# lmcinnes/pynndescent

Measured on AMD Instinct MI355X. Metric: index build: points indexed/sec (recall@10 vs brute force reported alongside), higher is better.
Workload: dtype f32

## Files before the change

### pynndescent_amd/csrc/rpforest.hip

```cpp
#include <atomic>
#include <chrono>

#include "common.h"
#include "state.h"

#define RP_EPS 1e-8f

static constexpr int SCAN_ITEMS = 8;
static constexpr int SCAN_BLOCK = 256;
static constexpr int SCAN_TILE = SCAN_ITEMS * SCAN_BLOCK;

__global__ void k_forest_init(int32_t *__restrict__ perm, int32_t *__restrict__ pos_seg, uint8_t *__restrict__ leaf_flag,
                              int32_t *__restrict__ inv, int64_t n, int64_t P, int splittable) {
    int64_t g = (int64_t)blockIdx.x * blockDim.x + threadIdx.x;
    if (g >= P) return;
    int64_t t = g / n;
    int64_t i = g - t * n;
    perm[g] = (int32_t)i;
    inv[g] = splittable ? (int32_t)t : -1;
    pos_seg[g] = splittable ? (int32_t)t : -1;
    leaf_flag[g] = (!splittable && i == 0) ? 1 : 0;
}
__global__ void k_forest_init_segs(int32_t *__restrict__ seg_start, int32_t *__restrict__ seg_len, int n_trees,
                                   int64_t n) {
// ... 1027 lines not shown
                    const float band = rp_band(xnorm, rx, hnorm, rh);
                    if (RP_IN_BAND(m, band)) {
                        const float4 *h4 = (const float4 *)(node_hf + (int64_t)node[u] * hs);
                        float e = 0.0f;
#pragma unroll
                        for (int q = 0; q < NC; q++) {
                            const int c = sub + 4 * q;
                            e = rp_dot4f(xa[q], h4[2 * c], e);
                            e = rp_dot4f(xb[q], h4[2 * c + 1], e);
                        }
                        m = rp_quad_sum(e) + off;
                    }
                    const int64_t slot = (int64_t)(t0 + u) * n + i;
                    int side;
                    if (fabsf(m) < RP_EPS) side = (int)(nnd_hash3(seed ^ 0x5bd1e995u, (uint32_t)slot, (uint32_t)depth) & 1u);
                    else side = m > 0.0f ? 0 : 1;
                    const int nxt = (int)(side ? meta[u].w : meta[u].z);
                    if (nxt <= -2) {
                        if (sub == 0) {
                            const int cell = -2 - nxt;
                            cell_of[slot] = cell;
                            rk[u] = atomicAdd(&cell_count[cell], 1);
                        }
                        node[u] = -1;
                    } else {
                        node[u] = nxt;
                    }
                }
            }
            if (sub == 0) {
#pragma unroll
                for (int u = 0; u < TB; u++)
                    if (t0 + u < n_trees) rank_of[(int64_t)(t0 + u) * n + i] = rk[u];
            }
        }
    }
}

#define RP_GLOBAL_TAG 0x40000000

__global__ __launch_bounds__(256) void k_top_heap(const unsigned char *__restrict__ pack, int rec, int dp, const int32_t *__restrict__ roots,
                                                  int L1, unsigned char *__restrict__ top_rec, int32_t *__restrict__ top_node,
                                                  int32_t *__restrict__ bucket_root) {
    __shared__ int32_t hn[256];
    const int t = blockIdx.x, nslots = 1 << L1, r16 = rec >> 4;
    if (threadIdx.x == 0) {
        hn[0] = -1;
        hn[1] = roots[t];
    }
    __syncthreads();
    for (int l = 0; l < L1; l++) {
        for (int sl = (1 << l) + threadIdx.x; sl < (2 << l); sl += blockDim.x) {
            const int nd = hn[sl];
            int c0 = -1, c1 = -1;
            if (nd >= 0) {
                const uint4 meta = *(const uint4 *)(pack + (int64_t)nd * rec + 2 * dp);
                c0 = (int)meta.z;
                c1 = (int)meta.w;
            }
            hn[2 * sl] = c0 >= 0 ? c0 : -1;
            hn[2 * sl + 1] = c1 >= 0 ? c1 : -1;
        }
        __syncthreads();
    }
    for (int q = threadIdx.x; q < nslots * r16; q += blockDim.x) {
        const int sl = q / r16, wd = q - sl * r16;
        const int nd = hn[sl];
        if (nd >= 0) ((uint4 *)(top_rec + (size_t)t * nslots * rec))[q] = ((const uint4 *)(pack + (int64_t)nd * rec))[wd];
    }
    for (int sl = threadIdx.x; sl < nslots; sl += blockDim.x) {
        top_node[t * nslots + sl] = hn[sl];
        bucket_root[t * nslots + sl] = hn[nslots + sl];
    }
}

__device__ __forceinline__ float rp_pair_sum(float v) {
    return v + __int_as_float(__builtin_amdgcn_update_dpp(0, __float_as_int(v), 0xB1, 0xF, 0xF, false));
}
template <int NC>
__device__ __forceinline__ float rp_exact_pair(const float *__restrict__ xrow, const float *__restrict__ h, int sub) {
    const float4 *x4 = (const float4 *)xrow;
    const float4 *h4 = (const float4 *)h;
    float ea = 0.0f, eb = 0.0f;
#pragma unroll
    for (int q = 0; q < NC; q++) {
        const int c = sub + 4 * q, c2 = sub + 2 + 4 * q;
        ea = rp_dot4f(x4[2 * c], h4[2 * c], ea);
        ea = rp_dot4f(x4[2 * c + 1], h4[2 * c + 1], ea);
        eb = rp_dot4f(x4[2 * c2], h4[2 * c2], eb);
        eb = rp_dot4f(x4[2 * c2 + 1], h4[2 * c2 + 1], eb);
    }
    ea = rp_pair_sum(ea);
    eb = rp_pair_sum(eb);
    return ea + eb;
}

template <int NC>
__global__ __launch_bounds__(1024) void k_route_top(const float *__restrict__ xp, const uint16_t *__restrict__ xh,
                                                    const float2 *__restrict__ nr, int metric, int dp, int64_t n, int64_t row_lo,
                                                    int64_t nrows, int tg0, int tgn, int L1, const unsigned char *__restrict__ top_rec,
                                                    const int32_t *__restrict__ top_node, const float *__restrict__ node_hf, int hs,
                                                    uint32_t seed, int32_t *__restrict__ cell_count, int32_t *__restrict__ cell_of,
                                                    int32_t *__restrict__ rank_of, int32_t *__restrict__ code,
                                                    int32_t *__restrict__ bucket_count, const float *__restrict__ scal) {
    extern __shared__ __attribute__((aligned(16))) unsigned char top_tab[];
    constexpr int NC2 = 2 * NC;
    const int rec = 2 * dp + 16, nslots = 1 << L1;
    const float inv_s2 = scal[1];
    int32_t *hist = (int32_t *)(top_tab + (size_t)tgn * nslots * rec);
    int32_t *tnode = hist + tgn * nslots;
    {
        const uint4 *src = (const uint4 *)(top_rec + (size_t)tg0 * nslots * rec);
        uint4 *dst = (uint4 *)top_tab;
        const int total = tgn * nslots * (rec >> 4);
        for (int q = threadIdx.x; q < total; q += blockDim.x) dst[q] = src[q];
        for (int q = threadIdx.x; q < tgn * nslots; q += blockDim.x) {
            hist[q] = 0;
            tnode[q] = top_node[tg0 * nslots + q];
        }
    }
    __syncthreads();
    const int sub = threadIdx.x & 1;
    const int ppb = blockDim.x >> 1;
    for (int64_t r0 = (int64_t)blockIdx.x * ppb; r0 < nrows; r0 += (int64_t)gridDim.x * ppb) {
        const int64_t r = r0 + (threadIdx.x >> 1);
        const bool on = r < nrows;
        const int64_t i = row_lo + (on ? r : 0);
        uint4 xq[NC2];
        {
            const uint4 *row = (const uint4 *)(xh + i * dp);
#pragma unroll
            for (int q = 0; q < NC2; q++) xq[q] = row[sub + 2 * q];
        }
        const float2 nrv = nr[i];
        const float xnorm = nnd_metric_unit(metric) ? nrv.x : sqrtf(nrv.x);
        const float bA = nrv.y + RP_ACC * xnorm, bB = xnorm + nrv.y;
        for (int tl = 0; tl < tgn; tl++) {
            const int t = tg0 + tl;
            const int64_t slot = (int64_t)t * n + i;
            int hidx = 1, rk = 0;
            bool fin = false;
            for (int depth = 0; depth < L1; depth++) {
                if (!__ballot(!fin)) break;
                const uint4 *r8 = (const uint4 *)(top_tab + ((size_t)tl * nslots + (fin ? 1 : hidx)) * rec);
                uint4 p[NC2];
#pragma unroll
                for (int q = 0; q < NC2; q++) p[q] = r8[sub + 2 * q];
                const uint4 meta = r8[dp >> 3];
                float acc = 0.0f;
#pragma unroll
                for (int q = 0; q < NC2; q++) acc = rp_dot8(xq[q], p[q], acc);
                if (fin) continue;
                const float off = __uint_as_float(meta.x), hnorm = __uint_as_float(meta.y & 0xFFFF0000u), rh = __uint_as_float(meta.y << 16);
                float m = rp_pair_sum(acc) * inv_s2 + off;
                const float band = hnorm * bA + rh * bB + RP_EPS;
                if (RP_IN_BAND(m, band))
                    m = rp_exact_pair<NC>(xp + i * dp, node_hf + (int64_t)tnode[tl * nslots + hidx] * hs, sub) + off;
                int side;
                if (fabsf(m) < RP_EPS) side = (int)(nnd_hash3(seed ^ 0x5bd1e995u, (uint32_t)slot, (uint32_t)depth) & 1u);
                else side = m > 0.0f ? 0 : 1;
                const int nxt = (int)(side ? meta.w : meta.z);
                if (nxt <= -2) {
                    if (sub == 0 && on) {
                        const int cell = -2 - nxt;
                        cell_of[(int64_t)t * nrows + r] = cell;
                        rk = atomicAdd(&cell_count[cell], 1);
                    }
                    fin = true;
                } else {
                    hidx = 2 * hidx + side;
                }
            }
            if (sub == 0 && on) {
                const int64_t o = (int64_t)t * nrows + r;
                if (fin) {
                    rank_of[o] = rk;
                    code[o] = -1;
                } else {
                    const int b = hidx - nslots;
                    code[o] = t * nslots + b;
                    atomicAdd(&hist[tl * nslots + b], 1);
                }
            }
        }
    }
    __syncthreads();
    for (int q = threadIdx.x; q < tgn * nslots; q += blockDim.x)
        if (hist[q]) atomicAdd(&bucket_count[tg0 * nslots + q], hist[q]);
}

__global__ __launch_bounds__(256) void k_bucket_prefix(const int32_t *__restrict__ bucket_count, int nb, int chunk,
                                                       int32_t *__restrict__ bucket_start, int2 *__restrict__ items,
                                                       int32_t *__restrict__ n_items, int max_items) {
    __shared__ int pa[256], pi[256];
    const int per = (nb + 255) / 256;
    const int b0 = threadIdx.x * per < nb ? threadIdx.x * per : nb, b1 = b0 + per < nb ? b0 + per : nb;
    int sa = 0, si = 0;
    for (int b = b0; b < b1; b++) {
        const int c = bucket_count[b];
        sa += c;
        si += (c + chunk - 1) / chunk;
    }
    pa[threadIdx.x] = sa;
    pi[threadIdx.x] = si;
    __syncthreads();
    if (threadIdx.x == 0) {
        int ra = 0, ri = 0;
        for (int q = 0; q < 256; q++) {
            const int va = pa[q], vi = pi[q];
            pa[q] = ra;
            pi[q] = ri;
            ra += va;
            ri += vi;
        }
        bucket_start[nb] = ra;
        n_items[0] = ri < max_items ? ri : max_items;
    }
    __syncthreads();
    int ra = pa[threadIdx.x], ri = pi[threadIdx.x];
    for (int b = b0; b < b1; b++) {
        const int c = bucket_count[b];
        bucket_start[b] = ra;
        ra += c;
        const int nc = (c + chunk - 1) / chunk;
        for (int j = 0; j < nc; j++)
            if (ri + j < max_items) items[ri + j] = make_int2(b, j);
        ri += nc;
    }
}

__global__ __launch_bounds__(256) void k_bucket_scatter(const int32_t *__restrict__ code, int64_t nrows, int64_t row_lo, int L1,
                                                        const int32_t *__restrict__ bucket_start, int32_t *__restrict__ bucket_cursor,
                                                        int32_t *__restrict__ bucket_rows, const float2 *__restrict__ nr, int metric,
                                                        uint32_t *__restrict__ bucket_ab) {
    __shared__ int cnt[256], base[256];
    const int t = blockIdx.y, nslots = 1 << L1;
    for (int q = threadIdx.x; q < nslots; q += 256) cnt[q] = 0;
    __syncthreads();
    const int64_t r0 = (int64_t)blockIdx.x * 4096;
    int myc[16], myr[16];
#pragma unroll
    for (int it = 0; it < 16; it++) {
        const int64_t r = r0 + it * 256 + threadIdx.x;
        const int c = r < nrows ? code[(int64_t)t * nrows + r] : -1;
        myc[it] = c;
        myr[it] = c >= 0 ? atomicAdd(&cnt[c - t * nslots], 1) : 0;
    }
    __syncthreads();
    for (int q = threadIdx.x; q < nslots; q += 256) base[q] = cnt[q] ? atomicAdd(&bucket_cursor[t * nslots + q], cnt[q]) : 0;
    __syncthreads();
#pragma unroll
    for (int it = 0; it < 16; it++) {
        const int c = myc[it];
        if (c < 0) continue;
        const int64_t r = r0 + it * 256 + threadIdx.x;
        const int at = bucket_start[c] + base[c - t * nslots] + myr[it];
        bucket_rows[at] = (int32_t)(row_lo + r);
        const float2 nrv = nr[row_lo + r];
        const float xnm = nnd_metric_unit(metric) ? nrv.x : sqrtf(nrv.x);
        bucket_ab[at] = (rp_bf16_up(nrv.y + RP_ACC * xnm) << 16) | rp_bf16_up(xnm + nrv.y);
    }
}

__global__ __launch_bounds__(64) void k_bucket_tables(const unsigned char *__restrict__ pack, int rec, int dp,
                                                      const int32_t *__restrict__ bucket_root, int R, int32_t *__restrict__ bt_cnt,
                                                      int32_t *__restrict__ bt_node, int32_t *__restrict__ bt_child,
                                                      unsigned char *__restrict__ bt_rec, int32_t *__restrict__ bt_cell) {
    const int b = blockIdx.x, lane = nnd_lane();
    int32_t *nodes = bt_node + (size_t)b * R;
    int32_t *child = bt_child + (size_t)b * R * 2;
    int32_t *cells = bt_cell + (size_t)b * (R + 8);
    const int root = bucket_root[b];
    if (root < 0) {
        if (lane == 0) bt_cnt[b] = 0;
        return;
    }
    int ccount = 0;
    __shared__ int32_t q_nodes[1024];
    if (lane == 0) q_nodes[0] = root;
    int count = 1, lb = 0, le = 1;
    nnd_wave_lds_sync();
    while (lb < le) {
        for (int i0 = lb; i0 < le; i0 += 64) {
            const int idx = i0 + lane;
            int c0 = -1, c1 = -1;
            if (idx < le) {
                const uint4 meta = *(const uint4 *)(pack + (int64_t)q_nodes[idx] * rec + 2 * dp);
                c0 = (int)meta.z;
                c1 = (int)meta.w;
            }
            const unsigned long long m0 = __ballot(idx < le && c0 >= 0), m1 = __ballot(idx < le && c1 >= 0);
            const int p0 = count + nnd_prefix_popc(m0), p1 = count + __popcll(m0) + nnd_prefix_popc(m1);
            const unsigned long long z0 = __ballot(idx < le && c0 <= -2), z1 = __ballot(idx < le && c1 <= -2);
            const int l0 = ccount + nnd_prefix_popc(z0), l1 = ccount + __popcll(z0) + nnd_prefix_popc(z1);
            ccount += __popcll(z0) + __popcll(z1);
            if (idx < le) {
                int k0 = c0, k1 = c1;
                if (c0 <= -2) { cells[l0] = -2 - c0; k0 = -2 - l0; }
                if (c1 <= -2) { cells[l1] = -2 - c1; k1 = -2 - l1; }
                if (c0 >= 0) {
                    if (p0 < R) { q_nodes[p0] = c0; k0 = p0; } else k0 = c0 + RP_GLOBAL_TAG;
                }
                if (c1 >= 0) {
                    if (p1 < R) { q_nodes[p1] = c1; k1 = p1; } else k1 = c1 + RP_GLOBAL_TAG;
                }
                child[2 * idx] = k0;
                child[2 * idx + 1] = k1;
            }
            count += __popcll(m0) + __popcll(m1);
            if (count > R) count = R;
            nnd_wave_lds_sync();
        }
        lb = le;
        le = count;
    }
    for (int i = lane; i < count; i += 64) nodes[i] = q_nodes[i];
    if (lane == 0) bt_cnt[b] = count;
    __threadfence_block();
    const int r16 = rec >> 4;
    uint4 *dst = (uint4 *)(bt_rec + (size_t)b * R * rec);
    for (int q = lane; q < count * r16; q += 64) {
        const int sl = q / r16, wd = q - sl * r16;
        uint4 v = ((const uint4 *)(pack + (int64_t)q_nodes[sl] * rec))[wd];
        if (wd == r16 - 1) {
            v.z = (uint32_t)child[2 * sl];
            v.w = (uint32_t)child[2 * sl + 1];
        }
        dst[q] = v;
    }
}

template <int NC>
__global__ __launch_bounds__(1024) void k_route_bucket(const float *__restrict__ xp, const uint16_t *__restrict__ xh,
                                                      const float2 *__restrict__ nr, int metric, int dp, int64_t n, int64_t row_lo,
                                                      int64_t nrows, int L1, int chunk, const unsigned char *__restrict__ pack,
                                                      const float *__restrict__ node_hf, int hs, const int2 *__restrict__ items,
                                                      const int32_t *__restrict__ n_items, const int32_t *__restrict__ bucket_start,
                                                      const int32_t *__restrict__ bucket_rows, const uint32_t *__restrict__ bucket_ab, int R,
                                                      const int32_t *__restrict__ bt_cnt, const int32_t *__restrict__ bt_node,
                                                      const unsigned char *__restrict__ bt_rec, const int32_t *__restrict__ bt_cell, uint32_t seed, int32_t *__restrict__ cell_count,
                                                      int32_t *__restrict__ cell_of, int32_t *__restrict__ rank_of,
                                                      const float *__restrict__ scal) {
    extern __shared__ __attribute__((aligned(16))) unsigned char sub_tab[];
    constexpr int NC2 = 2 * NC;
    const int rec = 2 * dp + 16, r16 = rec >> 4;
    const float inv_s2 = scal[1];
    int32_t *lcnt = (int32_t *)(sub_tab + (size_t)R * rec);
    int32_t *lbase = lcnt + (R + 8);
    int32_t *lcell = lbase + (R + 8);
    uint32_t *rowbuf = (uint32_t *)(lcell + (R + 8));
    const int sub = threadIdx.x & 1, ppb = blockDim.x >> 1, pair = threadIdx.x >> 1;
    const int ni = n_items[0];
#ifndef NND_ROUTE_CONTIG
    const int item0 = (int)blockIdx.x, item1 = ni, istep = (int)gridDim.x;
#else
    const int per = (ni + (int)gridDim.x - 1) / (int)gridDim.x;
    const int item0 = (int)blockIdx.x * per, item1 = item0 + per < ni ? item0 + per : ni, istep = 1;
#endif
    int cur_b = -1;
    for (int item = item0; item < item1; item += istep) {
        const int2 it = items[item];
        const int b = it.x;
        if (b != cur_b) {
            __syncthreads();
            const int cnt = bt_cnt[b];
            const uint4 *src = (const uint4 *)(bt_rec + (size_t)b * R * rec);
            for (int q = threadIdx.x; q < cnt * r16; q += blockDim.x) ((uint4 *)sub_tab)[q] = src[q];
            for (int q = threadIdx.x; q < R + 8; q += blockDim.x) {
                lcnt[q] = 0;
                lcell[q] = q <= cnt ? bt_cell[(size_t)b * (R + 8) + q] : 0;
            }
            cur_b = b;
            __syncthreads();
        }
        const int t = b >> L1;
        const int base = bucket_start[b] + it.y * chunk;
        int cnt_rows = bucket_start[b + 1] - base;
        if (cnt_rows > chunk) cnt_rows = chunk;
        for (int r0 = 0; r0 < cnt_rows; r0 += ppb) {
            const int idx = r0 + pair;
            const bool on = idx < cnt_rows;
            const int64_t pi = bucket_rows[base + (on ? idx : 0)];
            const uint32_t ab = bucket_ab[base + (on ? idx : 0)];
            uint4 xq[NC2];
            {
                const uint4 *row = (const uint4 *)(xh + pi * dp);
#pragma unroll
                for (int q = 0; q < NC2; q++) xq[q] = row[sub + 2 * q];
            }
            const float bA = __uint_as_float(ab & 0xFFFF0000u), bB = __uint_as_float(ab << 16);
            const int64_t slot = (int64_t)t * n + pi;
            int cur = on ? 0 : -1;
            int rk = -1;
            for (int depth = L1;; depth++) {
                if (!__ballot(cur >= 0)) break;
                uint4 p[NC2], meta;
                const bool glob = cur >= RP_GLOBAL_TAG;
                if (glob) {
                    const uint4 *r8 = (const uint4 *)(pack + (int64_t)(cur - RP_GLOBAL_TAG) * rec);
#pragma unroll
                    for (int q = 0; q < NC2; q++) p[q] = r8[sub + 2 * q];
                    meta = r8[dp >> 3];
                    if ((int)meta.z >= 0) meta.z += RP_GLOBAL_TAG;
                    if ((int)meta.w >= 0) meta.w += RP_GLOBAL_TAG;
                } else {
                    const uint4 *r8 = (const uint4 *)(sub_tab + (size_t)(cur >= 0 ? cur : 0) * rec);
#pragma unroll
                    for (int q = 0; q < NC2; q++) p[q] = r8[sub + 2 * q];
                    meta = r8[dp >> 3];
                }
                float acc = 0.0f;
#pragma unroll
                for (int q = 0; q < NC2; q++) acc = rp_dot8(xq[q], p[q], acc);
                if (cur < 0) continue;
                const float off = __uint_as_float(meta.x), hnorm = __uint_as_float(meta.y & 0xFFFF0000u), rh = __uint_as_float(meta.y << 16);
                float m = rp_pair_sum(acc) * inv_s2 + off;
                const float band = hnorm * bA + rh * bB + RP_EPS;
                if (RP_IN_BAND(m, band)) {
                    const int nd = glob ? cur - RP_GLOBAL_TAG : bt_node[(size_t)b * R + cur];
                    m = rp_exact_pair<NC>(xp + pi * dp, node_hf + (int64_t)nd * hs, sub) + off;
                }
                int side;
                if (fabsf(m) < RP_EPS) side = (int)(nnd_hash3(seed ^ 0x5bd1e995u, (uint32_t)slot, (uint32_t)depth) & 1u);
                else side = m > 0.0f ? 0 : 1;
                const int nxt = (int)(side ? meta.w : meta.z);
                if (nxt <= -2) {
                    if (sub == 0) {
                        const int cell = -2 - nxt;
                        if (glob) {
                            const int64_t o = (int64_t)t * nrows + (pi - row_lo);
                            cell_of[o] = cell;
                            rank_of[o] = atomicAdd(&cell_count[cell], 1);
                        } else {
                            rk = (cell << 16) | atomicAdd(&lcnt[cell], 1);
                        }
                    }
                    cur = -1;
                } else {
                    cur = nxt;
                }
            }
            if (sub == 0 && on) rowbuf[idx] = (uint32_t)rk;
        }
        __syncthreads();
        for (int q = threadIdx.x; q < R + 8; q += blockDim.x) {
            const int c = lcnt[q];
            if (c) {
                lbase[q] = atomicAdd(&cell_count[lcell[q]], c);
                lcnt[q] = 0;
            }
        }
        __syncthreads();
        for (int idx = threadIdx.x; idx < cnt_rows; idx += blockDim.x) {
            const uint32_t v = rowbuf[idx];
            if (v == 0xFFFFFFFFu) continue;
            const int lc = (int)(v >> 16);
            const int64_t o = (int64_t)t * nrows + (bucket_rows[base + idx] - row_lo);
            cell_of[o] = lcell[lc];
            rank_of[o] = lbase[lc] + (int)(v & 0xFFFFu);
        }
        __syncthreads();
    }
}

__global__ void k_cell_depths(const uint8_t *__restrict__ leaf_flag, const int32_t *__restrict__ leafscan,
                              const int32_t *__restrict__ leaf_depth, int64_t ps, int32_t *__restrict__ cell_depth) {
    const int64_t g = (int64_t)blockIdx.x * blockDim.x + threadIdx.x;
    if (g < ps && leaf_flag[g]) cell_depth[leafscan[g]] = leaf_depth[g];
}

__global__ void k_cell_lists(const int32_t *__restrict__ cell_count, const int32_t *__restrict__ cell_start,
                             const int32_t *__restrict__ cell_depth, int n_cells, int fin_small, int fin_max,
                             int32_t *__restrict__ small_list, int32_t *__restrict__ fin_start, int32_t *__restrict__ fin_len,
                             int32_t *__restrict__ fin_depth, int32_t *__restrict__ big_start, int32_t *__restrict__ big_len,
                             int32_t *__restrict__ big_depth, int64_t list_stride,
                             long long *__restrict__ counts ) {
    const int c = blockIdx.x * blockDim.x + threadIdx.x;
    const int len = c < n_cells ? cell_count[c] : 0;
    const int cls = len <= 0 ? -1 : (len <= fin_small ? 2 : (len <= fin_max ? 0 : 1));
#pragma unroll
    for (int k = 0; k < 3; k++) {
        const unsigned long long m = __ballot(cls == k);
        if (!m) continue;
        long long base = 0;
        if (nnd_lane() == __builtin_ctzll(m)) base = (long long)atomicAdd((unsigned long long *)&counts[k], (unsigned long long)__popcll(m));
        base = ((long long)__shfl((int)(base >> 32), __builtin_ctzll(m), 64) << 32) | (unsigned)__shfl((int)base, __builtin_ctzll(m), 64);
        if (cls == k) {
            const int64_t idx = base + nnd_prefix_popc(m);
            int32_t *st = k == 2 ? small_list : (k == 0 ? fin_start : big_start);
            int32_t *ln = k == 2 ? small_list + list_stride : (k == 0 ? fin_len : big_len);
            int32_t *dp_ = k == 2 ? small_list + 2 * list_stride : (k == 0 ? fin_depth : big_depth);
            st[idx] = cell_start[c];
            ln[idx] = len;
            dp_[idx] = cell_depth[c];
        }
    }
}

__global__ void k_place(const int32_t *__restrict__ cell_of, const int32_t *__restrict__ rank_of,
                        const int32_t *__restrict__ cell_start, int64_t nrows, int64_t row_lo, int32_t *__restrict__ perm) {
    const int64_t r = (int64_t)blockIdx.x * blockDim.x + threadIdx.x;
    if (r >= nrows) return;
    const int64_t slot = (int64_t)blockIdx.y * nrows + r;
    perm[cell_start[cell_of[slot]] + rank_of[slot]] = (int32_t)(row_lo + r);
}

enum forest_rc { FOREST_OK = 0, FOREST_ERROR = 1, FOREST_FALLBACK = 2 };
static forest_rc forest_fallback(const char *reason) {
    if (nnd_knob("NND_FOREST_DEBUG")) fprintf(stderr, "forest: fallback: %s\n", reason);
    return FOREST_FALLBACK;
}
#define FOREST_HIP_CHECK(expr) NND_HIP_CHECK_AS(expr, #expr, FOREST_ERROR)

static forest_rc run_scan(nnd_ctx *ctx, int mode, const int32_t *pos_seg, uint8_t *bytes, int32_t *total_dev, int64_t P, int64_t n,
                          const int32_t *perm = nullptr) {
    int nb = (int)((P + SCAN_TILE - 1) / SCAN_TILE);
    hipLaunchKernelGGL(k_scan_reduce, dim3(nb), dim3(SCAN_BLOCK), 0, ctx->stream, mode, pos_seg, bytes, P, ctx->scan_blk, perm,
                       ctx->side_pt, n);
    hipLaunchKernelGGL(k_scan_apply<true>, dim3(nb), dim3(SCAN_BLOCK), 0, ctx->stream, mode == 2 ? 0 : mode, pos_seg, bytes, P,
                       ctx->scan_blk, ctx->scan_out, total_dev);
    FOREST_HIP_CHECK(hipGetLastError());
    return FOREST_OK;
}

static forest_rc scan_i32_inplace(nnd_ctx *ctx, int32_t *data, int64_t n, int32_t *total_dev) {
    if (n <= SCAN_TILE) {
        hipLaunchKernelGGL(k_scan_blocks, dim3(1), dim3(256), 0, ctx->stream, data, (int)n, total_dev);
    } else {
        const int nb = (int)((n + SCAN_TILE - 1) / SCAN_TILE);
        hipLaunchKernelGGL(k_scan_i32_reduce, dim3(nb), dim3(SCAN_BLOCK), 0, ctx->stream, data, n, ctx->scan_blk);
        hipLaunchKernelGGL(k_scan_blocks, dim3(1), dim3(256), 0, ctx->stream, ctx->scan_blk, nb, total_dev);
        hipLaunchKernelGGL(k_scan_i32_apply, dim3(nb), dim3(SCAN_BLOCK), 0, ctx->stream, data, n, ctx->scan_blk);
    }
    FOREST_HIP_CHECK(hipGetLastError());
    return FOREST_OK;
}

static forest_rc read_scan_total(nnd_ctx *ctx, int32_t *out) {
    FOREST_HIP_CHECK(hipMemcpyAsync(&ctx->h_pin->scan_total, nnd_scan_total(ctx), sizeof(int32_t), hipMemcpyDeviceToHost, ctx->stream));
    FOREST_HIP_CHECK(nnd_sync_spin(ctx));
    *out = ctx->h_pin->scan_total;
    return FOREST_OK;
}

// ... 239 lines not shown
static forest_rc launch_route(nnd_ctx *ctx, const rp_route_io &io, int n_top, int l_top) {
    auto kern = k_route<NC, TB>;
    const size_t smem = (size_t)n_top * (2 * ctx->dp + 16);
    static bool attr_dev[64] = {false};
    if (!attr_dev[ctx->p.device & 63]) {
        FOREST_HIP_CHECK(hipFuncSetAttribute((const void *)kern, hipFuncAttributeMaxDynamicSharedMemorySize, 72 * 1024));
        attr_dev[ctx->p.device & 63] = true;
    }
    int n_cu = 0;
    if (device_cus(ctx, &n_cu)) return FOREST_ERROR;
    int64_t blocks = (ctx->n + 127) / 128;
    if (blocks > 2 * (int64_t)n_cu) blocks = 2 * (int64_t)n_cu;
    hipLaunchKernelGGL(kern, dim3((unsigned)blocks), dim3(512), smem, ctx->stream, ctx->xp, ctx->nr2, ctx->p.metric, ctx->dp, ctx->n,
                       io.T, io.pack, io.hf, ctx->dp + 4, ctx->tree_seed, io.cell_count, io.cell_of, io.rank_of, n_top, l_top, ctx->mean + ctx->dp);
    FOREST_HIP_CHECK(hipGetLastError());
    return FOREST_OK;
}

static forest_rc route_plain(nnd_ctx *ctx, const rp_route_io &io, const forest_view &v) {
    const int dp = ctx->dp;
    int l_top = 0;
    while (l_top + 1 < (int)v.level_base.size() && v.level_base[l_top + 1] * (2 * dp + 16) <= 72 * 1024) l_top++;
    const int n_top = (int)v.level_base[l_top];
    switch (dp / 32) {
        case 1: return launch_route<1, 4>(ctx, io, n_top, l_top);
        case 2: return launch_route<2, 4>(ctx, io, n_top, l_top);
        case 3: return launch_route<3, 2>(ctx, io, n_top, l_top);
        case 4: return launch_route<4, 2>(ctx, io, n_top, l_top);
        case 5: return launch_route<5, 1>(ctx, io, n_top, l_top);
        case 6: return launch_route<6, 1>(ctx, io, n_top, l_top);
        case 7: return launch_route<7, 1>(ctx, io, n_top, l_top);
        case 8: return launch_route<8, 1>(ctx, io, n_top, l_top);
        default: break;
    }
    return FOREST_FALLBACK;
}

#ifndef NND_ROUTE_L1
#define NND_ROUTE_L1 6
#endif
#ifndef NND_ROUTE_CHUNK
#define NND_ROUTE_CHUNK 2048
#endif
#ifndef NND_ROUTE_RMAX
#define NND_ROUTE_RMAX 384
#endif

struct rp_route_geom {
    int L1, ns, nb, R, chunk, tg;
    int64_t max_items;
    size_t o_top_rec, o_top_node, o_bucket_root, o_bcount, o_bcursor, o_bstart, o_nitems, o_btcnt, o_btnode, o_btchild, o_btrec, o_btcell, o_items, total;
};
static rp_route_geom route_geometry(int dp, int T, int64_t nrows, int64_t n_cells) {
    rp_route_geom g;
    const int rec = 2 * dp + 16;
    g.L1 = NND_ROUTE_L1;
    if (g.L1 < 7 && n_cells / ((int64_t)T << g.L1) > NND_ROUTE_RMAX / 2) g.L1 = 7;
    g.ns = 1 << g.L1;
    g.nb = T * g.ns;
    int64_t r = 6 * n_cells / g.nb + 16;
    const int64_t r_lds = (int64_t)150 * 1024 / rec;
    if (r > NND_ROUTE_RMAX) r = NND_ROUTE_RMAX;
    if (r > r_lds) r = r_lds;
    g.R = (int)(r < 64 ? 64 : r);
    g.chunk = NND_ROUTE_CHUNK;
    g.tg = (int)((size_t)140 * 1024 / ((size_t)g.ns * (rec + 8)));
    if (g.tg < 1) g.tg = 1;
    if (g.tg > T) g.tg = T;
    g.max_items = (int64_t)g.nb + (int64_t)T * nrows / g.chunk + 1;
    size_t at = 0;
    auto take = [&](size_t bytes) { const size_t o = at; at += (bytes + 255) & ~(size_t)255; return o; };
    g.o_top_rec = take((size_t)g.nb * rec);
    g.o_top_node = take(sizeof(int32_t) * g.nb);
    g.o_bucket_root = take(sizeof(int32_t) * g.nb);
    g.o_bcount = take(sizeof(int32_t) * g.nb);
    g.o_bcursor = take(sizeof(int32_t) * g.nb);
    g.o_bstart = take(sizeof(int32_t) * (g.nb + 1));
    g.o_nitems = take(sizeof(int32_t) * 4);
    g.o_btcnt = take(sizeof(int32_t) * g.nb);
    g.o_btnode = take(sizeof(int32_t) * (size_t)g.nb * g.R);
    g.o_btchild = take(sizeof(int32_t) * (size_t)g.nb * g.R * 2);
    g.o_btrec = take((size_t)g.nb * g.R * rec);
    g.o_btcell = take(sizeof(int32_t) * (size_t)g.nb * (g.R + 8));
    g.o_items = take(sizeof(int2) * (size_t)g.max_items);
    g.total = at;
    return g;
}

template <int NC>
static forest_rc launch_route_coherent(nnd_ctx *ctx, const rp_route_io &io, const rp_route_geom &g) {
    const int dp = ctx->dp, rec = 2 * dp + 16, hs = dp + 4;
    unsigned char *ws = ctx->route_ws;
    unsigned char *top_rec = ws + g.o_top_rec;
    int32_t *top_node = (int32_t *)(ws + g.o_top_node), *bucket_root = (int32_t *)(ws + g.o_bucket_root);
    int32_t *bcount = (int32_t *)(ws + g.o_bcount), *bcursor = (int32_t *)(ws + g.o_bcursor), *bstart = (int32_t *)(ws + g.o_bstart);
    int32_t *n_items = (int32_t *)(ws + g.o_nitems), *bt_cnt = (int32_t *)(ws + g.o_btcnt), *bt_node = (int32_t *)(ws + g.o_btnode);
    int32_t *bt_child = (int32_t *)(ws + g.o_btchild);
    unsigned char *bt_rec = ws + g.o_btrec;
    int32_t *bt_cell = (int32_t *)(ws + g.o_btcell);
    int2 *items = (int2 *)(ws + g.o_items);
    auto ktop = k_route_top<NC>;
    auto kbkt = k_route_bucket<NC>;
    static bool attr_dev[64] = {false};
    if (!attr_dev[ctx->p.device & 63]) {
        FOREST_HIP_CHECK(hipFuncSetAttribute((const void *)ktop, hipFuncAttributeMaxDynamicSharedMemorySize, 160 * 1024));
        FOREST_HIP_CHECK(hipFuncSetAttribute((const void *)kbkt, hipFuncAttributeMaxDynamicSharedMemorySize, 160 * 1024));
        attr_dev[ctx->p.device & 63] = true;
    }
    int n_cu = 0;
    if (device_cus(ctx, &n_cu)) return FOREST_ERROR;
    FOREST_HIP_CHECK(hipMemsetAsync(bcount, 0, g.o_bstart - g.o_bcount, ctx->stream));
    hipLaunchKernelGGL(k_top_heap, dim3((unsigned)io.T), dim3(256), 0, ctx->stream, io.pack, rec, dp, io.roots, g.L1, top_rec, top_node,
                       bucket_root);
    hipLaunchKernelGGL(k_bucket_tables, dim3((unsigned)g.nb), dim3(64), 0, ctx->stream, io.pack, rec, dp, bucket_root, g.R, bt_cnt, bt_node,
                       bt_child, bt_rec, bt_cell);
    for (int tg0 = 0; tg0 < io.T; tg0 += g.tg) {
        const int tgn = io.T - tg0 < g.tg ? io.T - tg0 : g.tg;
        const size_t smem = (size_t)tgn * g.ns * (rec + 8);
        int64_t blocks = (io.nrows + 511) / 512;
        if (blocks > n_cu) blocks = n_cu;
        hipLaunchKernelGGL(ktop, dim3((unsigned)blocks), dim3(1024), smem, ctx->stream, ctx->xp, ctx->xh, ctx->nr2, ctx->p.metric, dp, ctx->n, io.row_lo,
                           io.nrows, tg0, tgn, g.L1, top_rec, top_node, io.hf, hs, ctx->tree_seed, io.cell_count, io.cell_of, io.rank_of,
                           io.code, bcount, ctx->mean + ctx->dp);
    }
    hipLaunchKernelGGL(k_bucket_prefix, dim3(1), dim3(256), 0, ctx->stream, bcount, g.nb, g.chunk, bstart, items, n_items, (int)g.max_items);
    hipLaunchKernelGGL(k_bucket_scatter, dim3((unsigned)((io.nrows + 4095) / 4096), (unsigned)io.T), dim3(256), 0, ctx->stream, io.code,
                       io.nrows, io.row_lo, g.L1, bstart, bcursor, io.bucket_rows, ctx->nr2, ctx->p.metric, (uint32_t *)io.bucket_ab);
    const size_t smem2 = (size_t)g.R * rec + sizeof(int32_t) * 3 * (size_t)(g.R + 8) + sizeof(uint32_t) * (size_t)g.chunk;
    int per_cu = 0;
    FOREST_HIP_CHECK(hipOccupancyMaxActiveBlocksPerMultiprocessor(&per_cu, (const void *)kbkt, 1024, smem2));
    if (per_cu < 1) per_cu = 1;
    int64_t blocks2 = (int64_t)n_cu * per_cu;
    if (blocks2 > g.max_items) blocks2 = g.max_items;
    hipLaunchKernelGGL(kbkt, dim3((unsigned)blocks2), dim3(1024), smem2, ctx->stream, ctx->xp, ctx->xh, ctx->nr2, ctx->p.metric, dp, ctx->n,
                       io.row_lo, io.nrows, g.L1, g.chunk, io.pack, io.hf, hs, items, n_items, bstart, io.bucket_rows, (const uint32_t *)io.bucket_ab, g.R, bt_cnt, bt_node,
                       bt_rec, bt_cell, ctx->tree_seed, io.cell_count, io.cell_of, io.rank_of, ctx->mean + ctx->dp);
    FOREST_HIP_CHECK(hipGetLastError());
    return FOREST_OK;
}

static forest_rc route_coherent(nnd_ctx *ctx, const rp_route_io &io) {
    const int dp = ctx->dp;
    if (dp % 32 != 0 || dp > 256 || io.T < 1 || io.T > NND_ROUTE_TREES_MAX) return FOREST_FALLBACK;
    const rp_route_geom g = route_geometry(dp, io.T, io.nrows, io.n_cells);
    if (g.total > ctx->route_ws_cap) {
        FOREST_HIP_CHECK(hipStreamSynchronize(ctx->stream));
        if (ctx->route_ws) { FOREST_HIP_CHECK(hipFree(ctx->route_ws)); ctx->route_ws = nullptr; }
        ctx->route_ws_cap = 0;
        FOREST_HIP_CHECK(hipMalloc((void **)&ctx->route_ws, g.total + g.total / 4));
        ctx->route_ws_cap = g.total + g.total / 4;
    }
    switch (dp / 32) {
        case 1: return launch_route_coherent<1>(ctx, io, g);
        case 2: return launch_route_coherent<2>(ctx, io, g);
        case 3: return launch_route_coherent<3>(ctx, io, g);
        case 4: return launch_route_coherent<4>(ctx, io, g);
        case 5: return launch_route_coherent<5>(ctx, io, g);
        case 6: return launch_route_coherent<6>(ctx, io, g);
        case 7: return launch_route_coherent<7>(ctx, io, g);
        case 8: return launch_route_coherent<8>(ctx, io, g);
        default: break;
    }
    return FOREST_FALLBACK;
}

__global__ void k_iota_i32(int32_t *__restrict__ out, int n, int base) {
    const int i = blockIdx.x * blockDim.x + threadIdx.x;
    if (i < n) out[i] = base + i;
}

static forest_rc forest_tops(nnd_ctx *ctx, forest_view &v, int32_t *n_cells_out) {
    forest_rc rc = forest_levels(ctx, v);
    if (rc) return rc;
    int32_t n_cells = 0;
    if ((rc = run_scan(ctx, 1, nullptr, ctx->leaf_flag, nnd_scan_total(ctx), v.P, v.rows.n)) || (rc = read_scan_total(ctx, &n_cells))) return rc;
    if (n_cells > ctx->cell_cap) return forest_fallback("the recorded trees have more cells than the cell tables hold");
    hipLaunchKernelGGL(k_cell_depths, dim3((unsigned)((v.P + 255) / 256)), dim3(256), 0, ctx->stream, ctx->leaf_flag, ctx->scan_out,
                       ctx->s_leaf_depth, v.P, ctx->cell_depth);
    FOREST_HIP_CHECK(hipGetLastError());
    *n_cells_out = n_cells;
    return FOREST_OK;
}

static forest_rc forest_place_finish(nnd_ctx *ctx, int32_t n_cells, int T, int64_t row_lo, int64_t nrows, const int32_t *cell_of,
                                     const int32_t *rank_of, int64_t P_used, rp_tree_map tm) {
    FOREST_HIP_CHECK(hipMemcpyAsync(ctx->cell_start, ctx->cell_count, sizeof(int32_t) * (size_t)n_cells, hipMemcpyDeviceToDevice, ctx->stream));
    if (scan_i32_inplace(ctx, ctx->cell_start, n_cells, nnd_scan_total(ctx))) return FOREST_ERROR;
    FOREST_HIP_CHECK(hipMemsetAsync(ctx->leaf_flag, 0, (size_t)P_used, ctx->stream));
    long long *counts = ctx->counters + CNT_FIN_COUNT;
    FOREST_HIP_CHECK(hipMemsetAsync(counts, 0, 3 * sizeof(long long), ctx->stream));
    const nnd_work_list fin = nnd_fin_list(ctx), big = nnd_big_list(ctx), small = nnd_small_list(ctx);
    hipLaunchKernelGGL(k_cell_lists, dim3((unsigned)((n_cells + 255) / 256)), dim3(256), 0, ctx->stream, ctx->cell_count, ctx->cell_start,
                       ctx->cell_depth, (int)n_cells, FIN_SMALL, FIN_MAX, small.start, fin.start, fin.len, fin.depth, big.start,
                       big.len, big.depth, small.len - small.start, counts);
    if (cell_of)
        hipLaunchKernelGGL(k_place, dim3((unsigned)((nrows + 255) / 256), (unsigned)T), dim3(256), 0, ctx->stream, cell_of, rank_of,
                           ctx->cell_start, nrows, row_lo, ctx->perm[0]);
    FOREST_HIP_CHECK(hipGetLastError());
    FOREST_HIP_CHECK(hipMemcpyAsync(&ctx->h_pin->n_big, ctx->counters + CNT_BIG_COUNT, 2 * sizeof(long long), hipMemcpyDeviceToHost, ctx->stream));
    FOREST_HIP_CHECK(nnd_sync_spin(ctx));
    const long long n_big = ctx->h_pin->n_big, n_small = ctx->h_pin->n_small;
    if (n_big > ctx->max_segs) return forest_fallback("more over-long cells than the big work list holds");
    if (launch_finishers(ctx, ctx->perm[0], ctx->perm[1], big, 0, n_big, n_small, tm)) return FOREST_ERROR;
    ctx->cur = 0;
    return FOREST_OK;
}

static forest_rc forest_by_routing(nnd_ctx *ctx, int *levels_out) {
    const int64_t n = ctx->n, P = ctx->P, M = ctx->s_m, Ps = (int64_t)ctx->p.n_trees * M;
    const int T = ctx->p.n_trees, dp = ctx->dp;
    hipLaunchKernelGGL(k_gather_sample, dim3((unsigned)((M + 15) / 16)), dim3(256), 0, ctx->stream, ctx->xp, ctx->xh, ctx->nr2,
                       dp, (int64_t)0, M, ctx->s_stride, ctx->tree_seed, ctx->xs, ctx->xsh, ctx->nr2s);
    static const int rec_fin = [] { const char *e = nnd_knob("NND_REC_FIN"); const int r = e ? atoi(e) : FIN_SMALL; return r <= FIN_SMALL ? FIN_SMALL : FIN_MAX; }();
    forest_view v{{ctx->xs, ctx->xsh, ctx->nr2s, M, ctx->cell_leaf}, Ps, rec_fin, true};
    int32_t n_cells = 0;
    forest_rc rc = forest_tops(ctx, v, &n_cells);
    if (rc) return rc;
// ... 286 lines not shown
```

Measured before the change: 52.65 million.

## Software-pipeline row and bucket-table loads in RP-forest routing kernels

```diff
diff --git a/pynndescent_amd/csrc/rpforest.hip b/pynndescent_amd/csrc/rpforest.hip
--- a/pynndescent_amd/csrc/rpforest.hip
+++ b/pynndescent_amd/csrc/rpforest.hip
@@ -1133,21 +1133,32 @@
     const float4 *x4 = (const float4 *)xrow;
     const float4 *h4 = (const float4 *)h;
     float ea = 0.0f, eb = 0.0f;
-#pragma unroll
-    for (int q = 0; q < NC; q++) {
-        const int c = sub + 4 * q, c2 = sub + 2 + 4 * q;
-        ea = rp_dot4f(x4[2 * c], h4[2 * c], ea);
-        ea = rp_dot4f(x4[2 * c + 1], h4[2 * c + 1], ea);
-        eb = rp_dot4f(x4[2 * c2], h4[2 * c2], eb);
-        eb = rp_dot4f(x4[2 * c2 + 1], h4[2 * c2 + 1], eb);
+#pragma unroll 1
+    for (int j = 0; j < 2 * NC; j++) {
+        const int c = sub + 2 * j;
+        float e = (j & 1) ? eb : ea;
+        e = rp_dot4f(x4[2 * c], h4[2 * c], e);
+        e = rp_dot4f(x4[2 * c + 1], h4[2 * c + 1], e);
+        if (j & 1) eb = e;
+        else ea = e;
     }
     ea = rp_pair_sum(ea);
     eb = rp_pair_sum(eb);
     return ea + eb;
 }
 
+__device__ __forceinline__ int rp_now(int v) {
+    asm volatile("v_mov_b32 %0, %1" : "=v"(v) : "v"(v));
+    return v;
+}
+__device__ __forceinline__ int rp_tid_now() { return rp_now((int)threadIdx.x); }
+
 template <int NC>
-__global__ __launch_bounds__(1024) void k_route_top(const float *__restrict__ xp, const uint16_t *__restrict__ xh,
+constexpr bool rp_route_two_rows() { return NC <= 4; }
+constexpr int RP_ROUTE_THREADS = 1024, RP_ROUTE_PPB = RP_ROUTE_THREADS / 2;
+
+template <int NC>
+__global__ __launch_bounds__(RP_ROUTE_THREADS) void k_route_top(const float *__restrict__ xp, const uint16_t *__restrict__ xh,
                                                     const float2 *__restrict__ nr, int metric, int dp, int64_t n, int64_t row_lo,
                                                     int64_t nrows, int tg0, int tgn, int L1, const unsigned char *__restrict__ top_rec,
                                                     const int32_t *__restrict__ top_node, const float *__restrict__ node_hf, int hs,
@@ -1164,51 +1175,54 @@
         const uint4 *src = (const uint4 *)(top_rec + (size_t)tg0 * nslots * rec);
         uint4 *dst = (uint4 *)top_tab;
         const int total = tgn * nslots * (rec >> 4);
-        for (int q = threadIdx.x; q < total; q += blockDim.x) dst[q] = src[q];
-        for (int q = threadIdx.x; q < tgn * nslots; q += blockDim.x) {
+        for (int q = threadIdx.x; q < total; q += RP_ROUTE_THREADS) dst[q] = src[q];
+        for (int q = threadIdx.x; q < tgn * nslots; q += RP_ROUTE_THREADS) {
             hist[q] = 0;
             tnode[q] = top_node[tg0 * nslots + q];
         }
     }
     __syncthreads();
+    constexpr bool TWO = rp_route_two_rows<NC>();
     const int sub = threadIdx.x & 1;
-    const int ppb = blockDim.x >> 1;
-    for (int64_t r0 = (int64_t)blockIdx.x * ppb; r0 < nrows; r0 += (int64_t)gridDim.x * ppb) {
+    constexpr int ppb = RP_ROUTE_PPB;
+    const int64_t rstep = (int64_t)gridDim.x * ppb;
+    auto load_row = [&](int64_t r0, uint4 (&x)[NC2], float2 &nrv) {
+        const int tid = rp_tid_now();
+        const int64_t r = r0 + (tid >> 1);
+        const int64_t i = row_lo + (r < nrows ? r : 0);
+        const uint4 *row = (const uint4 *)(xh + i * dp) + (tid & 1);
+#pragma unroll
+        for (int q = 0; q < NC2; q++) x[q] = row[2 * q];
+        nrv = nr[i];
+    };
+    int64_t r0 = (int64_t)blockIdx.x * ppb;
+    auto walk_rows = [&](uint4 (&xq)[NC2], float2 &nrv, uint4 (&xq_next)[TWO ? NC2 : 1], float2 &nrv_next) {
+        if constexpr (TWO) load_row(r0 + rstep, xq_next, nrv_next);
+        else load_row(r0, xq, nrv);
         const int64_t r = r0 + (threadIdx.x >> 1);
         const bool on = r < nrows;
-        const int64_t i = row_lo + (on ? r : 0);
-        uint4 xq[NC2];
-        {
-            const uint4 *row = (const uint4 *)(xh + i * dp);
-#pragma unroll
-            for (int q = 0; q < NC2; q++) xq[q] = row[sub + 2 * q];
-        }
-        const float2 nrv = nr[i];
+        const int ri = on ? (int)(r - r0) : (int)-r0;
         const float xnorm = nnd_metric_unit(metric) ? nrv.x : sqrtf(nrv.x);
         const float bA = nrv.y + RP_ACC * xnorm, bB = xnorm + nrv.y;
         for (int tl = 0; tl < tgn; tl++) {
             const int t = tg0 + tl;
-            const int64_t slot = (int64_t)t * n + i;
             int hidx = 1, rk = 0;
             bool fin = false;
             for (int depth = 0; depth < L1; depth++) {
                 if (!__ballot(!fin)) break;
                 const uint4 *r8 = (const uint4 *)(top_tab + ((size_t)tl * nslots + (fin ? 1 : hidx)) * rec);
-                uint4 p[NC2];
-#pragma unroll
-                for (int q = 0; q < NC2; q++) p[q] = r8[sub + 2 * q];
                 const uint4 meta = r8[dp >> 3];
                 float acc = 0.0f;
 #pragma unroll
-                for (int q = 0; q < NC2; q++) acc = rp_dot8(xq[q], p[q], acc);
+                for (int q = 0; q < NC2; q++) acc = rp_dot8(xq[q], r8[sub + 2 * q], acc);
                 if (fin) continue;
                 const float off = __uint_as_float(meta.x), hnorm = __uint_as_float(meta.y & 0xFFFF0000u), rh = __uint_as_float(meta.y << 16);
                 float m = rp_pair_sum(acc) * inv_s2 + off;
                 const float band = hnorm * bA + rh * bB + RP_EPS;
                 if (RP_IN_BAND(m, band))
-                    m = rp_exact_pair<NC>(xp + i * dp, node_hf + (int64_t)tnode[tl * nslots + hidx] * hs, sub) + off;
+                    m = rp_exact_pair<NC>(xp + (row_lo + r0 + rp_now(ri)) * dp, node_hf + (int64_t)tnode[tl * nslots + hidx] * hs, sub) + off;
                 int side;
-                if (fabsf(m) < RP_EPS) side = (int)(nnd_hash3(seed ^ 0x5bd1e995u, (uint32_t)slot, (uint32_t)depth) & 1u);
+                if (fabsf(m) < RP_EPS) side = (int)(nnd_hash3(seed ^ 0x5bd1e995u, (uint32_t)((int64_t)t * n + row_lo + r0 + rp_now(ri)), (uint32_t)depth) & 1u);
                 else side = m > 0.0f ? 0 : 1;
                 const int nxt = (int)(side ? meta.w : meta.z);
                 if (nxt <= -2) {
@@ -1234,14 +1248,27 @@
                 }
             }
         }
+        r0 += rstep;
+    };
+    uint4 xa[NC2], xb[TWO ? NC2 : 1];
+    float2 na, nb;
+    if constexpr (TWO) {
+        load_row(r0, xa, na);
+        while (r0 < nrows) {
+            walk_rows(xa, na, xb, nb);
+            if (r0 >= nrows) break;
+            walk_rows(xb, nb, xa, na);
+        }
+    } else {
+        while (r0 < nrows) walk_rows(xa, na, xb, nb);
     }
     __syncthreads();
-    for (int q = threadIdx.x; q < tgn * nslots; q += blockDim.x)
+    for (int q = threadIdx.x; q < tgn * nslots; q += RP_ROUTE_THREADS)
         if (hist[q]) atomicAdd(&bucket_count[tg0 * nslots + q], hist[q]);
 }
 
 __global__ __launch_bounds__(256) void k_bucket_prefix(const int32_t *__restrict__ bucket_count, int nb, int chunk,
-                                                       int32_t *__restrict__ bucket_start, int2 *__restrict__ items,
+                                                       int32_t *__restrict__ bucket_start, int4 *__restrict__ items,
                                                        int32_t *__restrict__ n_items, int max_items) {
     __shared__ int pa[256], pi[256];
     const int per = (nb + 255) / 256;
@@ -1272,10 +1299,10 @@
     for (int b = b0; b < b1; b++) {
         const int c = bucket_count[b];
         bucket_start[b] = ra;
-        ra += c;
         const int nc = (c + chunk - 1) / chunk;
         for (int j = 0; j < nc; j++)
-            if (ri + j < max_items) items[ri + j] = make_int2(b, j);
+            if (ri + j < max_items) items[ri + j] = make_int4(b, ra + j * chunk, c - j * chunk < chunk ? c - j * chunk : chunk, 0);
+        ra += c;
         ri += nc;
     }
 }
@@ -1381,11 +1408,42 @@
     }
 }
 
+struct rp_round {
+    int b, base, cnt, r0;
+    __device__ __forceinline__ bool valid() const { return cnt > 0; }
+    __device__ __forceinline__ bool last() const { return r0 + RP_ROUTE_PPB >= cnt; }
+};
+struct rp_round_iter {
+    const int4 *items;
+    int item, item1, istep, ni, r0;
+    int4 rec, rec_next;
+    __device__ __forceinline__ int4 fetch(int i) const { return items[i < ni ? i : ni - 1]; }
+    __device__ __forceinline__ void start(const int4 *items_, int item0, int item1_, int istep_, int ni_) {
+        items = items_, item = item0, item1 = item1_, istep = istep_, ni = ni_, r0 = 0;
+        rec = fetch(item);
+        rec_next = fetch(item + istep);
+    }
+    __device__ __forceinline__ rp_round next() {
+        const bool valid = item < item1;
+        const rp_round d = {rec.x, valid ? rec.y : 0, valid ? rec.z : 0, r0};
+        if (valid) {
+            r0 += RP_ROUTE_PPB;
+            if (d.last()) {
+                r0 = 0;
+                item += istep;
+                rec = rec_next;
+                rec_next = fetch(item + istep);
+            }
+        }
+        return d;
+    }
+};
+
 template <int NC>
-__global__ __launch_bounds__(1024) void k_route_bucket(const float *__restrict__ xp, const uint16_t *__restrict__ xh,
+__global__ __launch_bounds__(RP_ROUTE_THREADS) void k_route_bucket(const float *__restrict__ xp, const uint16_t *__restrict__ xh,
                                                       const float2 *__restrict__ nr, int metric, int dp, int64_t n, int64_t row_lo,
                                                       int64_t nrows, int L1, int chunk, const unsigned char *__restrict__ pack,
-                                                      const float *__restrict__ node_hf, int hs, const int2 *__restrict__ items,
+                                                      const float *__restrict__ node_hf, int hs, const int4 *__restrict__ items,
                                                       const int32_t *__restrict__ n_items, const int32_t *__restrict__ bucket_start,
                                                       const int32_t *__restrict__ bucket_rows, const uint32_t *__restrict__ bucket_ab, int R,
                                                       const int32_t *__restrict__ bt_cnt, const int32_t *__restrict__ bt_node,
@@ -1394,13 +1452,14 @@
                                                       const float *__restrict__ scal) {
     extern __shared__ __attribute__((aligned(16))) unsigned char sub_tab[];
     constexpr int NC2 = 2 * NC;
+    constexpr bool TWO = rp_route_two_rows<NC>();
     const int rec = 2 * dp + 16, r16 = rec >> 4;
     const float inv_s2 = scal[1];
     int32_t *lcnt = (int32_t *)(sub_tab + (size_t)R * rec);
     int32_t *lbase = lcnt + (R + 8);
     int32_t *lcell = lbase + (R + 8);
     uint32_t *rowbuf = (uint32_t *)(lcell + (R + 8));
-    const int sub = threadIdx.x & 1, ppb = blockDim.x >> 1, pair = threadIdx.x >> 1;
+    const int sub = threadIdx.x & 1, pair = threadIdx.x >> 1;
     const int ni = n_items[0];
 #ifndef NND_ROUTE_CONTIG
     const int item0 = (int)blockIdx.x, item1 = ni, istep = (int)gridDim.x;
@@ -1408,109 +1467,153 @@
     const int per = (ni + (int)gridDim.x - 1) / (int)gridDim.x;
     const int item0 = (int)blockIdx.x * per, item1 = item0 + per < ni ? item0 + per : ni, istep = 1;
 #endif
-    int cur_b = -1;
-    for (int item = item0; item < item1; item += istep) {
-        const int2 it = items[item];
-        const int b = it.x;
-        if (b != cur_b) {
+    if (item0 >= item1) return;
+    rp_round_iter it;
+    it.start(items, item0, item1, istep, ni);
+
+    auto load_ids = [&](const rp_round &d, int32_t &pi, uint32_t &ab) {
+        const int idx = d.r0 + pair;
+        const int at = d.base + (idx < d.cnt ? idx : 0);
+        pi = bucket_rows[at];
+        ab = bucket_ab[at];
+    };
+    auto gather = [&](uint4 (&x)[NC2], int32_t pi) {
+        const uint4 *row = (const uint4 *)(xh + (int64_t)pi * dp);
+#pragma unroll
+        for (int q = 0; q < NC2; q++) x[q] = row[sub + 2 * q];
+    };
+    auto fill_table = [&](int b, int cnt, int from) {
+        const uint4 *src = (const uint4 *)(bt_rec + (size_t)b * R * rec);
+        const int tid = rp_tid_now();
+        for (int q = from + tid; q < cnt * r16; q += RP_ROUTE_THREADS) ((uint4 *)sub_tab)[q] = src[q];
+        for (int q = tid; q < R + 8; q += RP_ROUTE_THREADS) {
+            lcnt[q] = 0;
+            lcell[q] = q <= cnt ? bt_cell[(size_t)b * (R + 8) + q] : 0;
+        }
+    };
+
+    rp_round d0 = it.next(), d1 = it.next();
+    int32_t pi0, pi1;
+    uint32_t ab0, ab1;
+    load_ids(d0, pi0, ab0);
+    load_ids(d1, pi1, ab1);
+    uint4 xa[NC2], xb[TWO ? NC2 : 1];
+    if constexpr (TWO) gather(xa, pi0);
+    fill_table(d0.b, bt_cnt[d0.b], 0);
+    __syncthreads();
+
+    auto round = [&](uint4 (&cur)[NC2], uint4 (&nxt)[TWO ? NC2 : 1]) {
+        const rp_round d2 = it.next();
+        int32_t pi2;
+        uint32_t ab2;
+        load_ids(d2, pi2, ab2);
+        if constexpr (TWO) gather(nxt, pi1);
+        else gather(cur, pi0);
+        const bool new_tab = d0.last() && d1.valid() && d1.b != d0.b;
+
+        const int b = d0.b, t = b >> L1, idx = d0.r0 + pair;
+        const bool on = idx < d0.cnt;
+        const float bA = __uint_as_float(ab0 & 0xFFFF0000u), bB = __uint_as_float(ab0 << 16);
+        int cur_n = on ? 0 : -1;
+        int rk = -1;
+        for (int depth = L1;; depth++) {
+            if (!__ballot(cur_n >= 0)) break;
+            uint4 meta;
+            float acc = 0.0f;
+            const bool glob = cur_n >= RP_GLOBAL_TAG;
+            if (glob) {
+                const uint4 *r8 = (const uint4 *)(pack + (int64_t)(cur_n - RP_GLOBAL_TAG) * rec);
+                meta = r8[dp >> 3];
+#pragma unroll
+                for (int q = 0; q < NC2; q++) acc = rp_dot8(cur[q], r8[sub + 2 * q], acc);
+                if ((int)meta.z >= 0) meta.z += RP_GLOBAL_TAG;
+                if ((int)meta.w >= 0) meta.w += RP_GLOBAL_TAG;
+            } else {
+                const uint4 *r8 = (const uint4 *)(sub_tab + (size_t)(cur_n >= 0 ? cur_n : 0) * rec);
+                meta = r8[dp >> 3];
+#pragma unroll
+                for (int q = 0; q < NC2; q++) acc = rp_dot8(cur[q], r8[sub + 2 * q], acc);
+            }
+            if (cur_n < 0) continue;
+            const float off = __uint_as_float(meta.x), hnorm = __uint_as_float(meta.y & 0xFFFF0000u), rh = __uint_as_float(meta.y << 16);
+            float m = rp_pair_sum(acc) * inv_s2 + off;
+            const float band = hnorm * bA + rh * bB + RP_EPS;
+            if (RP_IN_BAND(m, band)) {
+                const int nd = glob ? cur_n - RP_GLOBAL_TAG : bt_node[(size_t)b * R + cur_n];
+                m = rp_exact_pair<NC>(xp + (int64_t)rp_now(pi0) * dp, node_hf + (int64_t)nd * hs, sub) + off;
+            }
+            int side;
+            if (fabsf(m) < RP_EPS) side = (int)(nnd_hash3(seed ^ 0x5bd1e995u, (uint32_t)((int64_t)t * n + rp_now(pi0)), (uint32_t)depth) & 1u);
+            else side = m > 0.0f ? 0 : 1;
+            const int nxt_n = (int)(side ? meta.w : meta.z);
+            if (nxt_n <= -2) {
+                if (sub == 0) {
+                    const int cell = -2 - nxt_n;
+                    if (glob) {
+                        const int64_t o = (int64_t)t * nrows + (rp_now(pi0) - row_lo);
+                        cell_of[o] = cell;
+                        rank_of[o] = atomicAdd(&cell_count[cell], 1);
+                    } else {
+                        rk = (cell << 16) | atomicAdd(&lcnt[cell], 1);
+                    }
+                }
+                cur_n = -1;
+            } else {
+                cur_n = nxt_n;
+            }
+        }
+        if (sub == 0 && on) rowbuf[idx] = (uint32_t)rk;
+
+        if (d0.last()) {
+            const int tid = rp_tid_now();
+            const int tq0 = tid, tq1 = tid + RP_ROUTE_THREADS;
+            uint4 tw0 = make_uint4(0, 0, 0, 0), tw1 = make_uint4(0, 0, 0, 0);
+            int tcnt = 0;
+            if (new_tab) {
+                const uint4 *src = (const uint4 *)(bt_rec + (size_t)d1.b * R * rec);
+                tcnt = bt_cnt[d1.b];
+                if (tq0 < R * r16) tw0 = src[tq0];
+                if (tq1 < R * r16) tw1 = src[tq1];
+            }
             __syncthreads();
-            const int cnt = bt_cnt[b];
-            const uint4 *src = (const uint4 *)(bt_rec + (size_t)b * R * rec);
-            for (int q = threadIdx.x; q < cnt * r16; q += blockDim.x) ((uint4 *)sub_tab)[q] = src[q];
-            for (int q = threadIdx.x; q < R + 8; q += blockDim.x) {
-                lcnt[q] = 0;
-                lcell[q] = q <= cnt ? bt_cell[(size_t)b * (R + 8) + q] : 0;
-            }
-            cur_b = b;
+            for (int q = tid; q < R + 8; q += RP_ROUTE_THREADS) {
+                const int c = lcnt[q];
+                if (c) {
+                    lbase[q] = atomicAdd(&cell_count[lcell[q]], c);
+                    lcnt[q] = 0;
+                }
+            }
             __syncthreads();
-        }
-        const int t = b >> L1;
-        const int base = bucket_start[b] + it.y * chunk;
-        int cnt_rows = bucket_start[b + 1] - base;
-        if (cnt_rows > chunk) cnt_rows = chunk;
-        for (int r0 = 0; r0 < cnt_rows; r0 += ppb) {
-            const int idx = r0 + pair;
-            const bool on = idx < cnt_rows;
-            const int64_t pi = bucket_rows[base + (on ? idx : 0)];
-            const uint32_t ab = bucket_ab[base + (on ? idx : 0)];
-            uint4 xq[NC2];
-            {
-                const uint4 *row = (const uint4 *)(xh + pi * dp);
-#pragma unroll
-                for (int q = 0; q < NC2; q++) xq[q] = row[sub + 2 * q];
-            }
-            const float bA = __uint_as_float(ab & 0xFFFF0000u), bB = __uint_as_float(ab << 16);
-            const int64_t slot = (int64_t)t * n + pi;
-            int cur = on ? 0 : -1;
-            int rk = -1;
-            for (int depth = L1;; depth++) {
-                if (!__ballot(cur >= 0)) break;
-                uint4 p[NC2], meta;
-                const bool glob = cur >= RP_GLOBAL_TAG;
-                if (glob) {
-                    const uint4 *r8 = (const uint4 *)(pack + (int64_t)(cur - RP_GLOBAL_TAG) * rec);
-#pragma unroll
-                    for (int q = 0; q < NC2; q++) p[q] = r8[sub + 2 * q];
-                    meta = r8[dp >> 3];
-                    if ((int)meta.z >= 0) meta.z += RP_GLOBAL_TAG;
-                    if ((int)meta.w >= 0) meta.w += RP_GLOBAL_TAG;
-                } else {
-                    const uint4 *r8 = (const uint4 *)(sub_tab + (size_t)(cur >= 0 ? cur : 0) * rec);
-#pragma unroll
-                    for (int q = 0; q < NC2; q++) p[q] = r8[sub + 2 * q];
-                    meta = r8[dp >> 3];
-                }
-                float acc = 0.0f;
-#pragma unroll
-                for (int q = 0; q < NC2; q++) acc = rp_dot8(xq[q], p[q], acc);
-                if (cur < 0) continue;
-                const float off = __uint_as_float(meta.x), hnorm = __uint_as_float(meta.y & 0xFFFF0000u), rh = __uint_as_float(meta.y << 16);
-                float m = rp_pair_sum(acc) * inv_s2 + off;
-                const float band = hnorm * bA + rh * bB + RP_EPS;
-                if (RP_IN_BAND(m, band)) {
-                    const int nd = glob ? cur - RP_GLOBAL_TAG : bt_node[(size_t)b * R + cur];
-                    m = rp_exact_pair<NC>(xp + pi * dp, node_hf + (int64_t)nd * hs, sub) + off;
-                }
-                int side;
-                if (fabsf(m) < RP_EPS) side = (int)(nnd_hash3(seed ^ 0x5bd1e995u, (uint32_t)slot, (uint32_t)depth) & 1u);
-                else side = m > 0.0f ? 0 : 1;
-                const int nxt = (int)(side ? meta.w : meta.z);
-                if (nxt <= -2) {
-                    if (sub == 0) {
-                        const int cell = -2 - nxt;
-                        if (glob) {
-                            const int64_t o = (int64_t)t * nrows + (pi - row_lo);
-                            cell_of[o] = cell;
-                            rank_of[o] = atomicAdd(&cell_count[cell], 1);
-                        } else {
-                            rk = (cell << 16) | atomicAdd(&lcnt[cell], 1);
-                        }
-                    }
-                    cur = -1;
-                } else {
-                    cur = nxt;
-                }
-            }
-            if (sub == 0 && on) rowbuf[idx] = (uint32_t)rk;
-        }
-        __syncthreads();
-        for (int q = threadIdx.x; q < R + 8; q += blockDim.x) {
-            const int c = lcnt[q];
-            if (c) {
-                lbase[q] = atomicAdd(&cell_count[lcell[q]], c);
-                lcnt[q] = 0;
-            }
-        }
-        __syncthreads();
-        for (int idx = threadIdx.x; idx < cnt_rows; idx += blockDim.x) {
-            const uint32_t v = rowbuf[idx];
-            if (v == 0xFFFFFFFFu) continue;
-            const int lc = (int)(v >> 16);
-            const int64_t o = (int64_t)t * nrows + (bucket_rows[base + idx] - row_lo);
-            cell_of[o] = lcell[lc];
-            rank_of[o] = lbase[lc] + (int)(v & 0xFFFFu);
-        }
-        __syncthreads();
+            for (int j = tid; j < d0.cnt; j += RP_ROUTE_THREADS) {
+                const uint32_t v = rowbuf[j];
+                if (v == 0xFFFFFFFFu) continue;
+                const int lc = (int)(v >> 16);
+                const int64_t o = (int64_t)t * nrows + (bucket_rows[d0.base + j] - row_lo);
+                cell_of[o] = lcell[lc];
+                rank_of[o] = lbase[lc] + (int)(v & 0xFFFFu);
+            }
+            __syncthreads();
+            if (new_tab) {
+                if (tq0 < tcnt * r16) ((uint4 *)sub_tab)[tq0] = tw0;
+                if (tq1 < tcnt * r16) ((uint4 *)sub_tab)[tq1] = tw1;
+                fill_table(d1.b, tcnt, 2 * RP_ROUTE_THREADS);
+                __syncthreads();
+            }
+        }
+        d0 = d1, d1 = d2;
+        pi0 = pi1, ab0 = ab1;
+        pi1 = pi2, ab1 = ab2;
+    };
+    if constexpr (TWO) {
+        for (;;) {
+            round(xa, xb);
+            if (!d0.valid()) break;
+            round(xb, xa);
+            if (!d0.valid()) break;
+        }
+    } else {
+        do round(xa, xb);
+        while (d0.valid());
     }
 }
 
@@ -1916,7 +2019,7 @@
     g.o_btchild = take(sizeof(int32_t) * (size_t)g.nb * g.R * 2);
     g.o_btrec = take((size_t)g.nb * g.R * rec);
     g.o_btcell = take(sizeof(int32_t) * (size_t)g.nb * (g.R + 8));
-    g.o_items = take(sizeof(int2) * (size_t)g.max_items);
+    g.o_items = take(sizeof(int4) * (size_t)g.max_items);
     g.total = at;
     return g;
 }
@@ -1932,7 +2035,7 @@
     int32_t *bt_child = (int32_t *)(ws + g.o_btchild);
     unsigned char *bt_rec = ws + g.o_btrec;
     int32_t *bt_cell = (int32_t *)(ws + g.o_btcell);
-    int2 *items = (int2 *)(ws + g.o_items);
+    int4 *items = (int4 *)(ws + g.o_items);
     auto ktop = k_route_top<NC>;
     auto kbkt = k_route_bucket<NC>;
     static bool attr_dev[64] = {false};
@@ -1951,9 +2054,9 @@
     for (int tg0 = 0; tg0 < io.T; tg0 += g.tg) {
         const int tgn = io.T - tg0 < g.tg ? io.T - tg0 : g.tg;
         const size_t smem = (size_t)tgn * g.ns * (rec + 8);
-        int64_t blocks = (io.nrows + 511) / 512;
+        int64_t blocks = (io.nrows + RP_ROUTE_PPB - 1) / RP_ROUTE_PPB;
         if (blocks > n_cu) blocks = n_cu;
-        hipLaunchKernelGGL(ktop, dim3((unsigned)blocks), dim3(1024), smem, ctx->stream, ctx->xp, ctx->xh, ctx->nr2, ctx->p.metric, dp, ctx->n, io.row_lo,
+        hipLaunchKernelGGL(ktop, dim3((unsigned)blocks), dim3(RP_ROUTE_THREADS), smem, ctx->stream, ctx->xp, ctx->xh, ctx->nr2, ctx->p.metric, dp, ctx->n, io.row_lo,
                            io.nrows, tg0, tgn, g.L1, top_rec, top_node, io.hf, hs, ctx->tree_seed, io.cell_count, io.cell_of, io.rank_of,
                            io.code, bcount, ctx->mean + ctx->dp);
     }
@@ -1962,11 +2065,11 @@
                        io.nrows, io.row_lo, g.L1, bstart, bcursor, io.bucket_rows, ctx->nr2, ctx->p.metric, (uint32_t *)io.bucket_ab);
     const size_t smem2 = (size_t)g.R * rec + sizeof(int32_t) * 3 * (size_t)(g.R + 8) + sizeof(uint32_t) * (size_t)g.chunk;
     int per_cu = 0;
-    FOREST_HIP_CHECK(hipOccupancyMaxActiveBlocksPerMultiprocessor(&per_cu, (const void *)kbkt, 1024, smem2));
+    FOREST_HIP_CHECK(hipOccupancyMaxActiveBlocksPerMultiprocessor(&per_cu, (const void *)kbkt, RP_ROUTE_THREADS, smem2));
     if (per_cu < 1) per_cu = 1;
     int64_t blocks2 = (int64_t)n_cu * per_cu;
     if (blocks2 > g.max_items) blocks2 = g.max_items;
-    hipLaunchKernelGGL(kbkt, dim3((unsigned)blocks2), dim3(1024), smem2, ctx->stream, ctx->xp, ctx->xh, ctx->nr2, ctx->p.metric, dp, ctx->n,
+    hipLaunchKernelGGL(kbkt, dim3((unsigned)blocks2), dim3(RP_ROUTE_THREADS), smem2, ctx->stream, ctx->xp, ctx->xh, ctx->nr2, ctx->p.metric, dp, ctx->n,
                        io.row_lo, io.nrows, g.L1, g.chunk, io.pack, io.hf, hs, items, n_items, bstart, io.bucket_rows, (const uint32_t *)io.bucket_ab, g.R, bt_cnt, bt_node,
                        bt_rec, bt_cell, ctx->tree_seed, io.cell_count, io.cell_of, io.rank_of, ctx->mean + ctx->dp);
     FOREST_HIP_CHECK(hipGetLastError());
```

Result: slower. 51.94 million (-1.4%).
